# JuliaParallel/DistributedArrays.jl

Measured on AMD Instinct MI355X. Metric: sum(DArray) GB/s, higher is better.
Workload: dtype f64; 1 GPU; cfg2: sum(drand(Float64, 2^28)) per GPU, 1-D block distribution; per_gpu_elems=268435456, global_elems=268435456

## Files before the change

distributedarrays_jl_amd/csrc/abi.hip:

```cpp
#include "common.hpp"
#include <stdarg.h>
#include <stdio.h>
#include <stdlib.h>
#include <unistd.h>
#include <errno.h>
#include <time.h>

namespace da {

static State g_state;
State& st() { return g_state; }

char g_errbuf[1024] = "ok";

int set_err(int code, const char* fmt, ...) {
    va_list ap;
    va_start(ap, fmt);
    vsnprintf(g_errbuf, sizeof(g_errbuf), fmt, ap);
    va_end(ap);
    return code;
}

int ensure_scratch(size_t bytes) {
    if (st().scratch_bytes >= bytes) return 0;
    if (st().scratch) hipFree(st().scratch);
    st().scratch = nullptr;
    st().scratch_bytes = 0;
    DA_CHECK_HIP(hipMalloc(&st().scratch, bytes));
    st().scratch_bytes = bytes;
    return 0;
}

int ensure_partials(size_t bytes) {
    if (st().partials_bytes >= bytes) return 0;
    if (st().partials) hipFree(st().partials);
    st().partials = nullptr;
    st().partials_bytes = 0;
    DA_CHECK_HIP(hipMalloc(&st().partials, bytes));
    st().partials_bytes = bytes;
    return 0;
}

static ncclDataType_t nccl_dtype(int dtype) {
    switch (dtype) {
    case DA_F64: return ncclDouble;
    case DA_F32: return ncclFloat;
    default: return ncclInt64;
    }
}

static ncclRedOp_t nccl_redop(int redop) {
    switch (redop) {
    case DA_RED_ADD: return ncclSum;
    case DA_RED_MUL: return ncclProd;
    case DA_RED_MIN: return ncclMin;
    default: return ncclMax;
    }
}

}

using namespace da;

extern "C" {

static uint64_t round_sz(uint64_t nbytes);
static int pool_trim_locked();


int da_init(int device, int rank, int nranks, const char* rccl_uid_path) {
    if (st().inited) return 0;
    if (nranks < 1 || rank < 0 || rank >= nranks)
        return set_err(-2, "da_init: bad rank %d/%d", rank, nranks);
    DA_CHECK_HIP(hipSetDevice(device));
    DA_CHECK_HIP(hipStreamCreateWithFlags(&st().stream, hipStreamNonBlocking));
    DA_CHECK_HIP(hipStreamCreateWithFlags(&st().comm_stream,
                                          hipStreamNonBlocking));
    DA_CHECK_HIP(hipEventCreateWithFlags(&st().ev_main,
                                         hipEventDisableTiming));
    DA_CHECK_HIP(hipEventCreateWithFlags(&st().ev_comm,
                                         hipEventDisableTiming));
    DA_CHECK_HIP(hipMalloc(&st().red_ticket, sizeof(unsigned int)));
    DA_CHECK_HIP(hipMemset(st().red_ticket, 0, sizeof(unsigned int)));
    st().device = device;
    st().rank = rank;
    st().nranks = nranks;
    if (nranks > 1) {
        if (!rccl_uid_path)
            return set_err(-2, "da_init: nranks>1 needs a uid path");
        ncclUniqueId uid;
        if (rank == 0) {
            DA_CHECK_NCCL(ncclGetUniqueId(&uid));
            char tmp[1024];
            snprintf(tmp, sizeof(tmp), "%s.tmp", rccl_uid_path);
            FILE* f = fopen(tmp, "wb");
            if (!f) return set_err(-4, "da_init: cannot write %s", tmp);
            fwrite(&uid, sizeof(uid), 1, f);
            fclose(f);
            if (rename(tmp, rccl_uid_path) != 0)
                return set_err(-4, "da_init: rename failed: %s",
                               strerror(errno));
        } else {
            FILE* f = nullptr;
            for (int i = 0; i < 1200 && !f; ++i) {
                f = fopen(rccl_uid_path, "rb");
                if (!f) usleep(100000);
            }
            if (!f) return set_err(-4, "da_init: uid file never appeared");
            size_t got = fread(&uid, 1, sizeof(uid), f);
            fclose(f);
            if (got != sizeof(uid))
                return set_err(-4, "da_init: short uid file");
        }
        DA_CHECK_NCCL(ncclCommInitRank(&st().comm, nranks, uid, rank));
    }
    st().inited = true;
    return 0;
}

int da_shutdown(void) {
    if (!st().inited) return 0;
    if (st().comm) { ncclCommDestroy(st().comm); st().comm = nullptr; }
    if (st().scratch) { hipFree(st().scratch); st().scratch = nullptr; }
    if (st().partials) { hipFree(st().partials); st().partials = nullptr; }
    (void)copy_nd_release();
    st().scratch_bytes = st().partials_bytes = 0;
    {
        std::lock_guard<std::mutex> g(st().mem_mtx);
        for (auto& kv : st().allocs) (void)hipFree(kv.first);
        st().allocs.clear();
        st().bytes_in_use = 0;
        (void)pool_trim_locked();
    }
    if (st().red_ticket) { (void)hipFree(st().red_ticket);
                           st().red_ticket = nullptr; }
    if (st().ev_main) { (void)hipEventDestroy(st().ev_main); st().ev_main = nullptr; }
    if (st().ev_comm) { (void)hipEventDestroy(st().ev_comm); st().ev_comm = nullptr; }
    if (st().comm_stream) { (void)hipStreamDestroy(st().comm_stream);
                            st().comm_stream = nullptr; }
    if (st().stream) { (void)hipStreamDestroy(st().stream); st().stream = nullptr; }
    st().inited = false;
    return 0;
}

int da_rank(void) { return st().rank; }
int da_nranks(void) { return st().nranks; }


static uint64_t round_sz(uint64_t nbytes) {
    if (nbytes == 0) nbytes = 1;
    return (nbytes + 255) & ~(uint64_t)255;
}

static int pool_trim_locked() {
    for (auto& kv : st().pool)
        for (void* p : kv.second)
            if (hipFree(p) != hipSuccess)
                return set_err(-5, "da_pool_trim: hipFree failed");
    st().pool.clear();
    st().pool_bytes = 0;
    return 0;
}

int da_alloc(uint64_t nbytes, int dtype, void** chunk) {
    DA_REQUIRE_INIT();
    if (!chunk) return set_err(-3, "da_alloc: null out");
    (void)dtype;
    uint64_t sz = round_sz(nbytes);
    void* p = nullptr;
    {
        std::lock_guard<std::mutex> g(st().mem_mtx);
        auto it = st().pool.find(sz);
        if (it != st().pool.end() && !it->second.empty()) {
            p = it->second.back();
            it->second.pop_back();
            st().pool_bytes -= sz;
        }
    }
    if (!p) {
        hipError_t e = hipMalloc(&p, sz);
        if (e != hipSuccess) {
            std::lock_guard<std::mutex> g(st().mem_mtx);
            int rc = pool_trim_locked();
            if (rc) return rc;
            e = hipMalloc(&p, sz);
            if (e != hipSuccess)
                return set_err(-(1000 + (int)e), "da_alloc(%llu): %s",
                               (unsigned long long)sz,
                               hipGetErrorString(e));
        }
    }
    {
        std::lock_guard<std::mutex> g(st().mem_mtx);
        st().allocs[p] = sz;
        st().bytes_in_use += sz;
    }
    *chunk = p;
    return 0;
}

int da_free(void* chunk) {
    DA_REQUIRE_INIT();
    if (!chunk) return 0;
    std::lock_guard<std::mutex> g(st().mem_mtx);
    auto it = st().allocs.find(chunk);
    if (it == st().allocs.end())
        return set_err(-3, "da_free: unknown chunk %p", chunk);
    uint64_t sz = it->second;
    st().bytes_in_use -= sz;
    st().allocs.erase(it);
    st().pool[sz].push_back(chunk);
    st().pool_bytes += sz;
    return 0;
}

int da_pool_trim(void) {
    DA_REQUIRE_INIT();
    DA_CHECK_HIP(hipStreamSynchronize(st().stream));
    std::lock_guard<std::mutex> g(st().mem_mtx);
    return pool_trim_locked();
}

uint64_t da_pool_bytes(void) {
    std::lock_guard<std::mutex> g(st().mem_mtx);
    return st().pool_bytes;
}

uint64_t da_bytes_in_use(void) {
    std::lock_guard<std::mutex> g(st().mem_mtx);
    return st().bytes_in_use;
}

int da_h2d(void* chunk, const void* host, uint64_t nbytes) {
    DA_REQUIRE_INIT();
    DA_CHECK_HIP(hipMemcpyAsync(chunk, host, nbytes, hipMemcpyHostToDevice,
                                st().stream));
    DA_CHECK_HIP(hipStreamSynchronize(st().stream));
    return 0;
}

int da_d2h(const void* chunk, void* host, uint64_t nbytes) {
    DA_REQUIRE_INIT();
    DA_CHECK_HIP(hipMemcpyAsync(host, chunk, nbytes, hipMemcpyDeviceToHost,
                                st().stream));
    DA_CHECK_HIP(hipStreamSynchronize(st().stream));
    return 0;
}

int da_d2d(void* dst, const void* src, uint64_t nbytes) {
    DA_REQUIRE_INIT();
    DA_CHECK_HIP(hipMemcpyAsync(dst, src, nbytes, hipMemcpyDeviceToDevice,
                                st().stream));
    return 0;
}

int da_copy2d(void* dst, uint64_t dpitch, const void* src, uint64_t spitch,
              uint64_t width, uint64_t height) {
    DA_REQUIRE_INIT();
    DA_CHECK_HIP(hipMemcpy2DAsync(dst, dpitch, src, spitch, width, height,
                                  hipMemcpyDeviceToDevice, st().stream));
    return 0;
}

int da_copy_nd_plan(const uint64_t* dst_shape, const int64_t* dst_start,
                    const int64_t* dst_step, const int64_t* const* dst_idx,
                    const uint64_t* src_shape, const int64_t* src_start,
                    const int64_t* src_step, const int64_t* const* src_idx,
                    const uint64_t* count, int nd, int dtype) {
    return copy_nd_plan(dst_shape, dst_start, dst_step, dst_idx,
                        src_shape, src_start, src_step, src_idx,
                        count, nd, dtype);
}

int da_copy_nd(void* dst, const uint64_t* dst_shape, const int64_t* dst_start,
               const int64_t* dst_step, const int64_t* const* dst_idx,
               const void* src, const uint64_t* src_shape,
               const int64_t* src_start, const int64_t* src_step,
               const int64_t* const* src_idx,
               const uint64_t* count, int nd, int dtype) {
    DA_REQUIRE_INIT();
    return launch_copy_nd(dst, dst_shape, dst_start, dst_step, dst_idx,
                          src, src_shape, src_start, src_step, src_idx,
                          count, nd, dtype, st().stream);
}


int da_fill(void* chunk, double v, uint64_t n, int dtype) {
    DA_REQUIRE_INIT();
    return launch_fill(chunk, v, n, dtype, st().stream);
}

int da_rand(void* chunk, uint64_t n, int dtype, uint64_t seed, int kind,
            uint64_t offset) {
    DA_REQUIRE_INIT();
    return launch_rand(chunk, n, dtype, seed, kind, offset, st().stream);
}

int da_map(int opcode, void* dst, const void* src, uint64_t n, int dtype) {
    DA_REQUIRE_INIT();
    return launch_map(opcode, dst, src, n, dtype, st().stream);
}

int da_map2(int opcode, void* dst, const void* a, const void* b,
            uint64_t n, int dtype) {
    DA_REQUIRE_INIT();
    return launch_map2(opcode, dst, a, b, n, dtype, st().stream);
}

int da_map2_scalar(int opcode, void* dst, const void* src, double c,
                   int reverse, uint64_t n, int dtype) {
    DA_REQUIRE_INIT();
    return launch_map2_scalar(opcode, dst, src, c, reverse, n, dtype,
                              st().stream);
}

int da_bcast_fma(void* d, const void* a, const void* b, double c,
                 uint64_t n, int dtype) {
    DA_REQUIRE_INIT();
    return launch_bcast_fma(d, a, b, c, n, dtype, st().stream);
}

int da_expr(const int32_t* prog, int prog_len, void* dst,
            const uint64_t* dst_dims, int nd,
            void* const* srcs, const uint64_t* src_strides, int nsrcs,
            const double* consts, int nconsts, uint64_t n, int dtype) {
    DA_REQUIRE_INIT();
    return launch_expr(prog, prog_len, dst, dst_dims, nd, srcs,
                       src_strides, nsrcs, consts, nconsts, n, dtype,
                       st().stream);
}

int da_expr_jit_state(void) { return expr_jit_state(); }
const char* da_expr_jit_errstr(void) { return expr_jit_err(); }

int da_axpby(void* y, const void* x, double alpha, double beta,
             uint64_t n, int dtype) {
    DA_REQUIRE_INIT();
    return launch_axpby(y, x, alpha, beta, n, dtype, st().stream);
}

int da_add(void* dest, const void* src, double scale, uint64_t n, int dtype) {
    DA_REQUIRE_INIT();
    return launch_add(dest, src, scale, n, dtype, st().stream);
}

int da_scale(void* a, double s, uint64_t n, int dtype) {
    DA_REQUIRE_INIT();
    return launch_scale(a, s, n, dtype, st().stream);
}

int da_cast(void* dst, int dst_dtype, const void* src, int src_dtype,
            uint64_t n) {
    DA_REQUIRE_INIT();
    return launch_cast(dst, dst_dtype, src, src_dtype, n, st().stream);
}

int da_reduce(int mapop, int redop, const void* src, uint64_t n, int dtype,
              void* out) {
    DA_REQUIRE_INIT();
    return launch_reduce(mapop, redop, src, n, dtype, out, st().stream);
}

int da_count(int mapop, const void* src, uint64_t n, int dtype,
             int64_t* out) {
    DA_REQUIRE_INIT();
    return launch_count(mapop, src, n, dtype, out, st().stream);
}

int da_reduce_dims(int mapop, int redop, const void* src, uint64_t inner,
                   uint64_t axis, uint64_t outer, int dtype, void* dst) {
    DA_REQUIRE_INIT();
    return launch_reduce_dims(mapop, redop, src, inner, axis, outer,
                              dtype, dst, st().stream);
}

int da_allreduce(void* inout, int count, int dtype, int redop) {
    DA_REQUIRE_INIT();
    if (count <= 0) return set_err(-3, "da_allreduce: bad count");
    size_t bytes = (size_t)count * dtype_size(dtype);
    if (st().nranks == 1) return 0;
    int rc = ensure_scratch(bytes);
    if (rc) return rc;
    DA_CHECK_HIP(hipMemcpyAsync(st().scratch, inout, bytes,
                                hipMemcpyHostToDevice, st().stream));
    DA_CHECK_NCCL(ncclAllReduce(st().scratch, st().scratch, count,
                                nccl_dtype(dtype), nccl_redop(redop),
                                st().comm, st().stream));
    DA_CHECK_HIP(hipMemcpyAsync(inout, st().scratch, bytes,
                                hipMemcpyDeviceToHost, st().stream));
    DA_CHECK_HIP(hipStreamSynchronize(st().stream));
    return 0;
}


int da_gemm_f64(void* C, const void* A, const void* B,
                int64_t m, int64_t n, int64_t k,
                int64_t lda, int64_t ldb, int64_t ldc,
                double alpha, double beta) {
    DA_REQUIRE_INIT();
    return launch_gemm_f64(C, A, B, m, n, k, lda, ldb, ldc, alpha, beta,
                           st().stream);
}

int da_gemm_f32(void* C, const void* A, const void* B,
                int64_t m, int64_t n, int64_t k,
                int64_t lda, int64_t ldb, int64_t ldc,
                double alpha, double beta) {
    DA_REQUIRE_INIT();
    return launch_gemm_f32(C, A, B, m, n, k, lda, ldb, ldc, alpha, beta,
                           st().stream);
}

int da_gemm_i64(void* C, const void* A, const void* B,
                int64_t m, int64_t n, int64_t k,
                int64_t lda, int64_t ldb, int64_t ldc,
                int64_t alpha, int64_t beta) {
    DA_REQUIRE_INIT();
    return launch_gemm_i64(C, A, B, m, n, k, lda, ldb, ldc, alpha, beta,
                           st().stream);
}

int da_transpose(void* dst, const void* src, uint64_t m, uint64_t n,
                 int dtype) {
    DA_REQUIRE_INIT();
    return launch_transpose(dst, src, m, n, dtype, st().stream);
}

int da_diag_scale(void* a, uint64_t m, uint64_t n, const void* diag,
                  int side, int dtype) {
    DA_REQUIRE_INIT();
    return launch_diag_scale(a, m, n, diag, side, dtype, st().stream);
}

int dbg_mfma_probe_f64(const void* A, const void* B, void* out_c,
                       void* out_raw) {
    DA_REQUIRE_INIT();
    return dbg_mfma_probe_impl(DA_F64, A, B, out_c, out_raw, st().stream);
}
// ... 160 lines not shown
```

distributedarrays_jl_amd/csrc/common.hpp:

```cpp
#pragma once
#include <hip/hip_runtime.h>
#include <rccl/rccl.h>
#include <stdint.h>
#include <stdio.h>
#include <string.h>
#include <mutex>
#include <unordered_map>

#include "darray_hip.h"

namespace da {

struct State {
    bool inited = false;
    int device = 0;
    int rank = 0;
    int nranks = 1;
    hipStream_t stream = nullptr;
    hipStream_t comm_stream = nullptr;
    bool p2p_comm = false;
    hipEvent_t ev_main = nullptr, ev_comm = nullptr;
    ncclComm_t comm = nullptr;
    void* scratch = nullptr;
    size_t scratch_bytes = 0;
    void* partials = nullptr;
    size_t partials_bytes = 0;
    unsigned int* red_ticket = nullptr;
    std::mutex mem_mtx;
    std::unordered_map<void*, uint64_t> allocs;
    uint64_t bytes_in_use = 0;
    std::unordered_map<uint64_t, std::vector<void*>> pool;
    uint64_t pool_bytes = 0;
};

State& st();

extern char g_errbuf[1024];
int set_err(int code, const char* fmt, ...);

#define DA_CHECK_HIP(expr) do {                                          \
    hipError_t _e = (expr);                                              \
    if (_e != hipSuccess)                                                \
        return da::set_err(-(1000 + (int)_e), "%s:%d hip error: %s",     \
                           __FILE__, __LINE__, hipGetErrorString(_e));   \
} while (0)

#define DA_CHECK_NCCL(expr) do {                                         \
    ncclResult_t _e = (expr);                                            \
    if (_e != ncclSuccess)                                               \
        return da::set_err(-(2000 + (int)_e), "%s:%d rccl error: %s",    \
                           __FILE__, __LINE__, ncclGetErrorString(_e));  \
} while (0)

#define DA_REQUIRE_INIT() do {                                           \
    if (!da::st().inited)                                                \
        return da::set_err(-1, "libdarray_hip: da_init() not called");   \
} while (0)

inline size_t dtype_size(int dtype) {
    switch (dtype) {
        case DA_F64: return 8;
        case DA_F32: return 4;
        case DA_I64: return 8;
    }
    return 0;
}

int ensure_scratch(size_t bytes);
int ensure_partials(size_t bytes);

int launch_fill(void* chunk, double v, uint64_t n, int dtype, hipStream_t s);
int launch_rand(void* chunk, uint64_t n, int dtype, uint64_t seed, int kind,
                uint64_t offset, hipStream_t s);
int launch_map(int opcode, void* dst, const void* src, uint64_t n, int dtype,
               hipStream_t s);
int launch_map2(int opcode, void* dst, const void* a, const void* b,
                uint64_t n, int dtype, hipStream_t s);
int launch_bcast_fma(void* d, const void* a, const void* b, double c,
                     uint64_t n, int dtype, hipStream_t s);
int launch_map2_scalar(int opcode, void* dst, const void* src, double c,
                       int rev, uint64_t n, int dtype, hipStream_t s);
int launch_expr(const int32_t* prog, int plen, void* dst,
                const uint64_t* dst_dims, int nd,
                void* const* srcs, const uint64_t* src_strides, int nsrcs,
                const double* consts, int nconsts,
                uint64_t n, int dtype, hipStream_t s);
int launch_expr_jit(const int32_t* prog, int plen, void* dst,
                    const uint64_t* dst_dims, int nd,
                    void* const* srcs, const uint64_t* src_strides,
                    int nsrcs, const double* consts, int nconsts,
                    uint64_t n, int dtype, hipStream_t s);
int expr_jit_state();
const char* expr_jit_err();
int launch_transpose(void* dst, const void* src, uint64_t m, uint64_t n,
                     int dtype, hipStream_t s);
int launch_diag_scale(void* a, uint64_t m, uint64_t n, const void* diag,
                      int side, int dtype, hipStream_t s);
int launch_axpby(void* y, const void* x, double alpha, double beta,
                 uint64_t n, int dtype, hipStream_t s);
int launch_add(void* dest, const void* src, double scale, uint64_t n,
               int dtype, hipStream_t s);
int launch_scale(void* a, double s_, uint64_t n, int dtype, hipStream_t s);
int launch_cast(void* dst, int dst_dtype, const void* src, int src_dtype,
                uint64_t n, hipStream_t s);
int launch_reduce(int mapop, int redop, const void* src, uint64_t n,
                  int dtype, void* out_host, hipStream_t s);
int launch_count(int mapop, const void* src, uint64_t n, int dtype,
                 int64_t* out_host, hipStream_t s);
int launch_reduce_dims(int mapop, int redop, const void* src,
                       uint64_t inner, uint64_t axis, uint64_t outer,
                       int dtype, void* dst, hipStream_t s);
int launch_gemm_f64(void* C, const void* A, const void* B,
                    int64_t m, int64_t n, int64_t k,
                    int64_t lda, int64_t ldb, int64_t ldc,
                    double alpha, double beta, hipStream_t s);
int launch_gemm_i64(void* C, const void* A, const void* B,
                    int64_t m, int64_t n, int64_t k,
                    int64_t lda, int64_t ldb, int64_t ldc,
                    int64_t alpha, int64_t beta, hipStream_t s);
int launch_gemm_f32(void* C, const void* A, const void* B,
                    int64_t m, int64_t n, int64_t k,
                    int64_t lda, int64_t ldb, int64_t ldc,
                    double alpha, double beta, hipStream_t s);
int copy_nd_plan(const uint64_t* dst_shape, const int64_t* dst_start,
                 const int64_t* dst_step, const int64_t* const* dst_idx,
                 const uint64_t* src_shape, const int64_t* src_start,
                 const int64_t* src_step, const int64_t* const* src_idx,
                 const uint64_t* count, int nd, int dtype);
int launch_copy_nd(void* dst, const uint64_t* dst_shape,
                   const int64_t* dst_start, const int64_t* dst_step,
                   const int64_t* const* dst_idx,
                   const void* src, const uint64_t* src_shape,
                   const int64_t* src_start, const int64_t* src_step,
                   const int64_t* const* src_idx,
                   const uint64_t* count, int nd, int dtype, hipStream_t s);
int copy_nd_release();
int reduce_dims_variant(uint64_t inner, uint64_t axis, uint64_t outer);
int gemm_path(int64_t m, int64_t n, int64_t k);
int dbg_mfma_probe_impl(int dtype, const void* A, const void* B,
                        void* out_c, void* out_raw, hipStream_t s);

}
```

distributedarrays_jl_amd/csrc/kernels_reduce.hip:

```cpp
#include "common.hpp"
#include <stdlib.h>

namespace da {

constexpr int RTPB = 256;
constexpr int RMAXB = 8192;

static inline int reduce_grid(uint64_t want) {
    static int cap = -1;
    if (cap < 0) {
        const char* e = getenv("DA_RBLOCKS");
        cap = e ? atoi(e) : 2048;
        if (cap < 1 || cap > RMAXB) cap = 2048;
    }
    if (want < 1) want = 1;
    return (int)(want > (uint64_t)cap ? (uint64_t)cap : want);
}

static inline bool reduce_v4() {
    static int v = -1;
    if (v < 0) {
        const char* e = getenv("DA_RV4");
        v = e ? atoi(e) : 0;
    }
    return v == 1;
}

template <typename T> struct RedIdent {
    static __device__ __host__ T get(int redop) {
        switch (redop) {
        case DA_RED_ADD: return (T)0;
        case DA_RED_MUL: return (T)1;
        case DA_RED_MIN: return (T)INFINITY;
        case DA_RED_MAX: return (T)(-INFINITY);
        }
        return (T)0;
    }
};
template <> struct RedIdent<int64_t> {
    static __device__ __host__ int64_t get(int redop) {
        switch (redop) {
        case DA_RED_ADD: return 0;
        case DA_RED_MUL: return 1;
        case DA_RED_MIN: return INT64_MAX;
        case DA_RED_MAX: return INT64_MIN;
        }
        return 0;
    }
};

template <typename T>
__device__ __forceinline__ T red_comb(int redop, T a, T b) {
    switch (redop) {
    case DA_RED_ADD: return a + b;
    case DA_RED_MUL: return a * b;
    case DA_RED_MIN:
        return a != a ? a : (b != b ? b : (a < b ? a : b));
    case DA_RED_MAX:
        return a != a ? a : (b != b ? b : (a > b ? a : b));
    }
    return a;
}
__device__ __forceinline__ int64_t red_comb(int redop, int64_t a, int64_t b) {
    switch (redop) {
    case DA_RED_ADD: return (int64_t)((uint64_t)a + (uint64_t)b);
    case DA_RED_MUL: return (int64_t)((uint64_t)a * (uint64_t)b);
    case DA_RED_MIN: return a < b ? a : b;
    case DA_RED_MAX: return a > b ? a : b;
    }
    return a;
}

template <typename T>
__device__ __forceinline__ T mapf(int mapop, T x) {
    switch (mapop) {
    case DA_REDF_IDENTITY: return x;
    case DA_REDF_ABS: return fabs(x);
    case DA_REDF_ABS2: return x * x;
    case DA_REDF_ISNAN: return (T)(x != x ? 1 : 0);
    case DA_REDF_ISFINITE: return (T)(isfinite((double)x) ? 1 : 0);
    case DA_REDF_NONZERO: return (T)(x != (T)0 ? 1 : 0);
    }
    return x;
}
__device__ __forceinline__ int64_t mapf(int mapop, int64_t x) {
    switch (mapop) {
    case DA_REDF_IDENTITY: return x;
    case DA_REDF_ABS: return x < 0 ? (int64_t)(0ull - (uint64_t)x) : x;
    case DA_REDF_ABS2: return (int64_t)((uint64_t)x * (uint64_t)x);
    case DA_REDF_ISNAN: return 0;
    case DA_REDF_ISFINITE: return 1;
    case DA_REDF_NONZERO: return x != 0 ? 1 : 0;
    }
    return x;
}

template <typename T>
__device__ __forceinline__ T block_reduce(int redop, T v) {
    __shared__ T lds[RTPB / 64];
#pragma unroll
    for (int off = 32; off > 0; off >>= 1)
        v = red_comb(redop, v, (T)__shfl_down(v, off, 64));
    int wave = threadIdx.x / 64, lane = threadIdx.x % 64;
    if (lane == 0) lds[wave] = v;
    __syncthreads();
    if (wave == 0) {
        T w = lane < (RTPB / 64) ? lds[lane]
                                 : RedIdent<T>::get(redop);
#pragma unroll
        for (int off = 2; off > 0; off >>= 1)
            w = red_comb(redop, w, (T)__shfl_down(w, off, 64));
        return w;
    }
    return v;
}

template <typename T, int MOP = -1, int ROP = -1>
__global__ void reduce_stage1(int mapop, int redop, const T* __restrict__ src,
                              uint64_t n, T* __restrict__ partials) {
    if (MOP >= 0) mapop = MOP;
    if (ROP >= 0) redop = ROP;
    uint64_t i = (uint64_t)blockIdx.x * blockDim.x + threadIdx.x;
    uint64_t stride = (uint64_t)gridDim.x * blockDim.x;
    T acc = RedIdent<T>::get(redop);
    using V = T __attribute__((ext_vector_type(2)));
    uint64_t nv = n / 2;
    const V* sv = reinterpret_cast<const V*>(src);
    for (uint64_t j = i; j < nv; j += stride) {
        V v = sv[j];
        acc = red_comb(redop, acc, mapf<T>(mapop, (T)v.x));
        acc = red_comb(redop, acc, mapf<T>(mapop, (T)v.y));
    }
    for (uint64_t j = 2 * nv + i; j < n; j += stride)
        acc = red_comb(redop, acc, mapf<T>(mapop, src[j]));
    acc = block_reduce(redop, acc);
    if (threadIdx.x == 0) partials[blockIdx.x] = acc;
}

template <typename T, int MOP = -1, int ROP = -1>
__global__ void reduce_stage1_v4(int mapop, int redop,
                                 const T* __restrict__ src, uint64_t n,
                                 T* __restrict__ partials) {
    if (MOP >= 0) mapop = MOP;
    if (ROP >= 0) redop = ROP;
    uint64_t i = (uint64_t)blockIdx.x * blockDim.x + threadIdx.x;
    uint64_t stride = (uint64_t)gridDim.x * blockDim.x;
    T acc = RedIdent<T>::get(redop);
    using V = T __attribute__((ext_vector_type(4)));
    uint64_t nv = n / 4;
    const V* sv = reinterpret_cast<const V*>(src);
    for (uint64_t j = i; j < nv; j += stride) {
        V v = sv[j];
        acc = red_comb(redop, acc, mapf<T>(mapop, (T)v.x));
        acc = red_comb(redop, acc, mapf<T>(mapop, (T)v.y));
        acc = red_comb(redop, acc, mapf<T>(mapop, (T)v.z));
        acc = red_comb(redop, acc, mapf<T>(mapop, (T)v.w));
    }
    for (uint64_t j = 4 * nv + i; j < n; j += stride)
        acc = red_comb(redop, acc, mapf<T>(mapop, src[j]));
    acc = block_reduce(redop, acc);
    if (threadIdx.x == 0) partials[blockIdx.x] = acc;
}

template <typename T>
__global__ void reduce_fused(int mapop, int redop, const T* __restrict__ src,
                             uint64_t n, T* __restrict__ partials,
                             unsigned int* __restrict__ ticket,
                             T* __restrict__ out) {
    __shared__ int is_last;
    uint64_t i = (uint64_t)blockIdx.x * blockDim.x + threadIdx.x;
    uint64_t stride = (uint64_t)gridDim.x * blockDim.x;
    T acc = RedIdent<T>::get(redop);
    using V = T __attribute__((ext_vector_type(2)));
    uint64_t nv = n / 2;
    const V* sv = reinterpret_cast<const V*>(src);
    for (uint64_t j = i; j < nv; j += stride) {
        V v = sv[j];
        acc = red_comb(redop, acc, mapf<T>(mapop, (T)v.x));
        acc = red_comb(redop, acc, mapf<T>(mapop, (T)v.y));
    }
    for (uint64_t j = 2 * nv + i; j < n; j += stride)
        acc = red_comb(redop, acc, mapf<T>(mapop, src[j]));
    acc = block_reduce(redop, acc);
    if (threadIdx.x == 0) partials[blockIdx.x] = acc;
    __asm__ volatile("s_waitcnt vmcnt(0)" ::: "memory");
    __syncthreads();
    if (threadIdx.x == 0) {
        __builtin_amdgcn_fence(__ATOMIC_RELEASE, "agent");
        __asm__ volatile("s_waitcnt vmcnt(0)" ::: "memory");
        unsigned int t = __hip_atomic_fetch_add(
            ticket, 1u, __ATOMIC_RELAXED, __HIP_MEMORY_SCOPE_AGENT);
        is_last = (t == gridDim.x - 1);
    }
    __syncthreads();
    if (!is_last) return;
    if (threadIdx.x == 0)
        __builtin_amdgcn_fence(__ATOMIC_ACQUIRE, "agent");
    __syncthreads();
    T facc = RedIdent<T>::get(redop);
    for (unsigned int j = threadIdx.x; j < gridDim.x; j += blockDim.x)
        facc = red_comb(redop, facc, partials[j]);
    __syncthreads();
    facc = block_reduce(redop, facc);
    if (threadIdx.x == 0) {
        out[0] = facc;
        *ticket = 0;
    }
}

template <typename T>
__global__ void reduce_stage2(int redop, const T* __restrict__ partials,
                              int np, T* __restrict__ out) {
    T acc = RedIdent<T>::get(redop);
    for (int j = threadIdx.x; j < np; j += blockDim.x)
        acc = red_comb(redop, acc, partials[j]);
    acc = block_reduce(redop, acc);
    if (threadIdx.x == 0) out[0] = acc;
}

template <typename T>
static int do_reduce(int mapop, int redop, const T* src, uint64_t n,
                     void* out_host, hipStream_t s) {
    if (n == 0) {
        *(T*)out_host = RedIdent<T>::get(redop);
        return 0;
    }
    bool v4 = reduce_v4();
    uint64_t want = (n / (v4 ? 4 : 2) + RTPB - 1) / RTPB;
    int g = reduce_grid(want);
    int rc = ensure_partials((RMAXB + 1) * sizeof(double));
    if (rc) return rc;
    T* parts = (T*)st().partials;
    T* dout = (T*)((double*)st().partials + RMAXB);
    unsigned int* ticket = st().red_ticket;
    static int fused = -1;
    if (fused < 0) {
        const char* e = getenv("DA_RED_FUSED");
        fused = e ? atoi(e) : 0;
    }
    if (fused && !v4) {
        hipLaunchKernelGGL(reduce_fused<T>, dim3(g), dim3(RTPB), 0, s,
                           mapop, redop, src, n, parts, ticket, dout);
        DA_CHECK_HIP(hipGetLastError());
    } else {
        if (v4)
            hipLaunchKernelGGL((reduce_stage1_v4<T>), dim3(g), dim3(RTPB),
                               0, s, mapop, redop, src, n, parts);
        else if (mapop == DA_REDF_IDENTITY && redop == DA_RED_ADD)
            hipLaunchKernelGGL((reduce_stage1<T, DA_REDF_IDENTITY,
                                DA_RED_ADD>), dim3(g), dim3(RTPB), 0, s,
                               mapop, redop, src, n, parts);
        else if (mapop == DA_REDF_ABS2 && redop == DA_RED_ADD)
            hipLaunchKernelGGL((reduce_stage1<T, DA_REDF_ABS2,
                                DA_RED_ADD>), dim3(g), dim3(RTPB), 0, s,
                               mapop, redop, src, n, parts);
        else if (mapop == DA_REDF_ABS && redop == DA_RED_ADD)
            hipLaunchKernelGGL((reduce_stage1<T, DA_REDF_ABS,
                                DA_RED_ADD>), dim3(g), dim3(RTPB), 0, s,
                               mapop, redop, src, n, parts);
        else if (mapop == DA_REDF_IDENTITY && redop == DA_RED_MAX)
            hipLaunchKernelGGL((reduce_stage1<T, DA_REDF_IDENTITY,
                                DA_RED_MAX>), dim3(g), dim3(RTPB), 0, s,
                               mapop, redop, src, n, parts);
        else if (mapop == DA_REDF_IDENTITY && redop == DA_RED_MIN)
            hipLaunchKernelGGL((reduce_stage1<T, DA_REDF_IDENTITY,
                                DA_RED_MIN>), dim3(g), dim3(RTPB), 0, s,
                               mapop, redop, src, n, parts);
        else
            hipLaunchKernelGGL((reduce_stage1<T>), dim3(g), dim3(RTPB),
                               0, s, mapop, redop, src, n, parts);
        DA_CHECK_HIP(hipGetLastError());
        hipLaunchKernelGGL(reduce_stage2<T>, dim3(1), dim3(RTPB), 0, s,
                           redop, parts, g, dout);
        DA_CHECK_HIP(hipGetLastError());
    }
    DA_CHECK_HIP(hipMemcpyAsync(out_host, dout, sizeof(T),
                                hipMemcpyDeviceToHost, s));
    DA_CHECK_HIP(hipStreamSynchronize(s));
    return 0;
}

template <typename T>
__device__ __forceinline__ int64_t predf(int mapop, T x) {
    switch (mapop) {
    case DA_REDF_ISNAN: return x != x ? 1 : 0;
    case DA_REDF_ISFINITE: return isfinite((double)x) ? 1 : 0;
    }
    return x != (T)0 ? 1 : 0;
}
template <>
__device__ __forceinline__ int64_t predf<int64_t>(int mapop, int64_t x) {
    return mapf(mapop, x);
}

template <typename T>
__global__ void count_stage1(int mapop, const T* __restrict__ src,
                             uint64_t n, int64_t* __restrict__ partials) {
    uint64_t i = (uint64_t)blockIdx.x * blockDim.x + threadIdx.x;
    uint64_t stride = (uint64_t)gridDim.x * blockDim.x;
    int64_t acc = 0;
    using V = T __attribute__((ext_vector_type(2)));
    uint64_t nv = n / 2;
    const V* sv = reinterpret_cast<const V*>(src);
    for (uint64_t j = i; j < nv; j += stride) {
        V v = sv[j];
        acc += predf<T>(mapop, (T)v.x) + predf<T>(mapop, (T)v.y);
    }
    for (uint64_t j = 2 * nv + i; j < n; j += stride)
        acc += predf<T>(mapop, src[j]);
    acc = block_reduce(DA_RED_ADD, acc);
    if (threadIdx.x == 0) partials[blockIdx.x] = acc;
}

template <typename T>
static int do_count(int mapop, const T* src, uint64_t n, int64_t* out_host,
                    hipStream_t s) {
    int g = reduce_grid((n / 2 + RTPB - 1) / RTPB);
    int rc = ensure_partials((RMAXB + 1) * sizeof(double));
    if (rc) return rc;
    int64_t* parts = (int64_t*)st().partials;
    int64_t* dout = parts + RMAXB;
    hipLaunchKernelGGL(count_stage1<T>, dim3(g), dim3(RTPB), 0, s,
                       mapop, src, n, parts);
    DA_CHECK_HIP(hipGetLastError());
    hipLaunchKernelGGL(reduce_stage2<int64_t>, dim3(1), dim3(RTPB), 0, s,
                       (int)DA_RED_ADD, parts, g, dout);
    DA_CHECK_HIP(hipGetLastError());
    DA_CHECK_HIP(hipMemcpyAsync(out_host, dout, sizeof(int64_t),
                                hipMemcpyDeviceToHost, s));
    DA_CHECK_HIP(hipStreamSynchronize(s));
    return 0;
}

int launch_count(int mapop, const void* src, uint64_t n, int dtype,
                 int64_t* out_host, hipStream_t s) {
    if (mapop < DA_REDF_ISNAN || mapop > DA_REDF_NONZERO)
        return set_err(-3, "da_count: mapop %d is not a predicate", mapop);
    if (!out_host) return set_err(-3, "da_count: null out");
    if (dtype != DA_F64 && dtype != DA_F32 && dtype != DA_I64)
        return set_err(-3, "da_count: bad dtype %d", dtype);
    if (n == 0) { *out_host = 0; return 0; }
    switch (dtype) {
    case DA_F64: return do_count<double>(mapop, (const double*)src, n,
                                         out_host, s);
    case DA_F32: return do_count<float>(mapop, (const float*)src, n,
                                        out_host, s);
    }
    return do_count<int64_t>(mapop, (const int64_t*)src, n, out_host, s);
}

template <typename T, int MOP, int ROP>
__global__ void reduce_dims_threads(int mapop, int redop,
                                    const T* __restrict__ src,
                                    uint64_t inner, uint64_t axis,
                                    uint64_t outer, T* __restrict__ dst) {
    const int mop_ = MOP >= 0 ? MOP : mapop;
    const int rop_ = ROP >= 0 ? ROP : redop;
    uint64_t t = (uint64_t)blockIdx.x * blockDim.x + threadIdx.x;
    uint64_t stride = (uint64_t)gridDim.x * blockDim.x;
    uint64_t total = inner * outer;
    for (uint64_t e = t; e < total; e += stride) {
        uint64_t i = e % inner, o = e / inner;
        const T* p = src + i + o * inner * axis;
        T acc = RedIdent<T>::get(rop_);
        for (uint64_t a = 0; a < axis; ++a)
            acc = red_comb(rop_, acc, mapf(mop_, p[a * inner]));
        dst[i + o * inner] = acc;
    }
}

template <typename T, int MOP, int ROP>
__global__ void reduce_dims_waves(int mapop, int redop,
                                  const T* __restrict__ src,
                                  uint64_t inner, uint64_t axis,
                                  uint64_t outer, T* __restrict__ dst) {
    const int mop_ = MOP >= 0 ? MOP : mapop;
    const int rop_ = ROP >= 0 ? ROP : redop;
    uint64_t wid = ((uint64_t)blockIdx.x * blockDim.x + threadIdx.x) / 64;
    uint64_t nw = ((uint64_t)gridDim.x * blockDim.x) / 64;
    int lane = threadIdx.x & 63;
    uint64_t total = inner * outer;
    for (uint64_t e = wid; e < total; e += nw) {
        uint64_t i = e % inner, o = e / inner;
        const T* p = src + i + o * inner * axis;
        T acc = RedIdent<T>::get(rop_);
        for (uint64_t a = lane; a < axis; a += 64)
            acc = red_comb(rop_, acc, mapf(mop_, p[a * inner]));
#pragma unroll
        for (int off = 32; off > 0; off >>= 1)
            acc = red_comb(rop_, acc, (T)__shfl_down(acc, off, 64));
        if (lane == 0) dst[i + o * inner] = acc;
    }
}

template <typename T, int MOP, int ROP>
__global__ void reduce_dims_blocks(int mapop, int redop,
                                   const T* __restrict__ src,
                                   uint64_t inner, uint64_t axis,
                                   uint64_t outer, T* __restrict__ dst) {
    const int mop_ = MOP >= 0 ? MOP : mapop;
    const int rop_ = ROP >= 0 ? ROP : redop;
    uint64_t total = inner * outer;
    for (uint64_t e = blockIdx.x; e < total; e += gridDim.x) {
        uint64_t i = e % inner, o = e / inner;
        const T* p = src + i + o * inner * axis;
        T acc = RedIdent<T>::get(rop_);
        for (uint64_t a = threadIdx.x; a < axis; a += blockDim.x)
            acc = red_comb(rop_, acc, mapf(mop_, p[a * inner]));
        acc = block_reduce(rop_, acc);
        if (threadIdx.x == 0) dst[i + o * inner] = acc;
        __syncthreads();
    }
}

template <typename T, int MOP, int ROP>
__global__ void reduce_dims_slices1(int mapop, int redop,
                                    const T* __restrict__ src,
                                    uint64_t inner, uint64_t axis,
                                    int nb, T* __restrict__ partials) {
    const int mop_ = MOP >= 0 ? MOP : mapop;
    const int rop_ = ROP >= 0 ? ROP : redop;
    uint64_t o = blockIdx.z;
    const T* base = src + o * inner * axis;
    uint64_t row = (uint64_t)blockIdx.x * blockDim.x + threadIdx.x;
    if (row >= inner) return;
    uint64_t a0 = axis * blockIdx.y / nb;
    uint64_t a1 = axis * (blockIdx.y + 1) / nb;
    T acc = RedIdent<T>::get(rop_);
    for (uint64_t a = a0; a < a1; ++a)
        acc = red_comb(rop_, acc, mapf(mop_, base[row + a * inner]));
    partials[(o * nb + blockIdx.y) * inner + row] = acc;
}

template <typename T>
__global__ void reduce_dims_slices2(int redop, const T* __restrict__ partials,
                                    uint64_t inner, int nb,
                                    T* __restrict__ dst, uint64_t outer) {
    uint64_t e = (uint64_t)blockIdx.x * blockDim.x + threadIdx.x;
    uint64_t stride = (uint64_t)gridDim.x * blockDim.x;
    for (uint64_t t = e; t < inner * outer; t += stride) {
        uint64_t row = t % inner, o = t / inner;
        T acc = RedIdent<T>::get(redop);
        for (int b = 0; b < nb; ++b)
            acc = red_comb(redop, acc,
                           partials[(o * nb + b) * inner + row]);
        dst[row + o * inner] = acc;
    }
}

int reduce_dims_variant(uint64_t inner, uint64_t axis, uint64_t outer) {
    uint64_t total = inner * outer;
    if (total < 262144 && inner >= 64 && axis >= 64 && outer <= 64)
        return DA_DIMS_SLICES;
    if (total >= 262144 && inner >= 64)
        return DA_DIMS_THREADS;
    if (inner < 64 && axis >= 64 && total >= 16384)
        return DA_DIMS_WAVES;
    return DA_DIMS_BLOCKS;
}

template <typename T, int MOP, int ROP>
static int do_reduce_dims_t(int mapop, int redop, const T* src,
                            uint64_t inner, uint64_t axis, uint64_t outer,
                            T* dst, hipStream_t s) {
    uint64_t total = inner * outer;
    if (total == 0) return 0;
    const int variant = reduce_dims_variant(inner, axis, outer);
    if (variant == DA_DIMS_SLICES) {
        uint64_t row_tiles = (inner + RTPB - 1) / RTPB;
        int nb = (int)(2048 / row_tiles);
        if (nb < 1) nb = 1;
        if (nb > 64) nb = 64;
        if ((uint64_t)nb > axis) nb = (int)axis;
        int rc = ensure_partials((uint64_t)nb * inner * outer * sizeof(T));
        if (rc) return rc;
        T* parts = (T*)st().partials;
        dim3 g((inner + RTPB - 1) / RTPB, nb, outer);
        hipLaunchKernelGGL((reduce_dims_slices1<T, MOP, ROP>), g,
                           dim3(RTPB), 0, s,
                           mapop, redop, src, inner, axis, nb, parts);
        DA_CHECK_HIP(hipGetLastError());
        uint64_t want = (total + RTPB - 1) / RTPB;
        int g2 = (int)(want < 1 ? 1 : (want > 2048 ? 2048 : want));
        hipLaunchKernelGGL(reduce_dims_slices2<T>, dim3(g2), dim3(RTPB), 0,
                           s, redop, parts, inner, nb, dst, outer);
        DA_CHECK_HIP(hipGetLastError());
        return 0;
    }
    if (variant == DA_DIMS_THREADS) {
        uint64_t want = (total + RTPB - 1) / RTPB;
        int g = (int)(want < 1 ? 1 : (want > 8192 ? 8192 : want));
        hipLaunchKernelGGL((reduce_dims_threads<T, MOP, ROP>), dim3(g),
                           dim3(RTPB), 0,
                           s, mapop, redop, src, inner, axis, outer, dst);
    } else if (variant == DA_DIMS_WAVES) {
        uint64_t want = (total * 64 + RTPB - 1) / RTPB;
        int g = (int)(want < 1 ? 1 : (want > 8192 ? 8192 : want));
        hipLaunchKernelGGL((reduce_dims_waves<T, MOP, ROP>), dim3(g),
                           dim3(RTPB), 0,
                           s, mapop, redop, src, inner, axis, outer, dst);
    } else {
        int g = (int)(total < 1 ? 1 : (total > 8192 ? 8192 : total));
        hipLaunchKernelGGL((reduce_dims_blocks<T, MOP, ROP>), dim3(g),
                           dim3(RTPB), 0,
                           s, mapop, redop, src, inner, axis, outer, dst);
    }
    DA_CHECK_HIP(hipGetLastError());
    return 0;
}

template <typename T>
static int do_reduce_dims(int mapop, int redop, const T* src,
                          uint64_t inner, uint64_t axis, uint64_t outer,
                          T* dst, hipStream_t s) {
    if (redop == DA_RED_ADD) {
        if (mapop == DA_REDF_IDENTITY)
            return do_reduce_dims_t<T, DA_REDF_IDENTITY, DA_RED_ADD>(
                mapop, redop, src, inner, axis, outer, dst, s);
        if (mapop == DA_REDF_ABS2)
            return do_reduce_dims_t<T, DA_REDF_ABS2, DA_RED_ADD>(
                mapop, redop, src, inner, axis, outer, dst, s);
    }
    if (redop == DA_RED_MAX && mapop == DA_REDF_IDENTITY)
        return do_reduce_dims_t<T, DA_REDF_IDENTITY, DA_RED_MAX>(
            mapop, redop, src, inner, axis, outer, dst, s);
    if (redop == DA_RED_MIN && mapop == DA_REDF_IDENTITY)
        return do_reduce_dims_t<T, DA_REDF_IDENTITY, DA_RED_MIN>(
            mapop, redop, src, inner, axis, outer, dst, s);
    return do_reduce_dims_t<T, -1, -1>(mapop, redop, src, inner, axis,
                                       outer, dst, s);
}

int launch_reduce_dims(int mapop, int redop, const void* src,
                       uint64_t inner, uint64_t axis, uint64_t outer,
                       int dtype, void* dst, hipStream_t s) {
    if (mapop < 0 || mapop > DA_REDF_NONZERO || redop < 0 || redop > DA_RED_MAX)
        return set_err(-3, "da_reduce_dims: bad op (%d,%d)", mapop, redop);
    switch (dtype) {
    case DA_F64: return do_reduce_dims<double>(mapop, redop,
        (const double*)src, inner, axis, outer, (double*)dst, s);
    case DA_F32: return do_reduce_dims<float>(mapop, redop,
        (const float*)src, inner, axis, outer, (float*)dst, s);
    case DA_I64: return do_reduce_dims<int64_t>(mapop, redop,
        (const int64_t*)src, inner, axis, outer, (int64_t*)dst, s);
    }
    return set_err(-3, "da_reduce_dims: bad dtype %d", dtype);
}

int launch_reduce(int mapop, int redop, const void* src, uint64_t n,
                  int dtype, void* out_host, hipStream_t s) {
    if (mapop < 0 || mapop > DA_REDF_NONZERO || redop < 0 || redop > DA_RED_MAX)
        return set_err(-3, "da_reduce: bad op (%d,%d)", mapop, redop);
    switch (dtype) {
    case DA_F64: return do_reduce<double>(mapop, redop, (const double*)src,
                                          n, out_host, s);
    case DA_F32: return do_reduce<float>(mapop, redop, (const float*)src,
                                         n, out_host, s);
    case DA_I64: return do_reduce<int64_t>(mapop, redop, (const int64_t*)src,
                                           n, out_host, s);
    }
    return set_err(-3, "da_reduce: bad dtype %d", dtype);
}

}
```

Measured before the change: 6023 GB/s.

## Default to fused single-pass reduction with monotonic ticket and pinned host result

```diff
diff --git a/distributedarrays_jl_amd/csrc/abi.hip b/distributedarrays_jl_amd/csrc/abi.hip
--- a/distributedarrays_jl_amd/csrc/abi.hip
+++ b/distributedarrays_jl_amd/csrc/abi.hip
@@ -82,6 +82,11 @@
                                          hipEventDisableTiming));
     DA_CHECK_HIP(hipMalloc(&st().red_ticket, sizeof(unsigned int)));
     DA_CHECK_HIP(hipMemset(st().red_ticket, 0, sizeof(unsigned int)));
+    st().red_base = 0;
+    DA_CHECK_HIP(hipHostMalloc(&st().red_host, 16, hipHostMallocDefault));
+    memset(st().red_host, 0, 16);
+    DA_CHECK_HIP(hipHostGetDevicePointer(&st().red_host_dev,
+                                         st().red_host, 0));
     st().device = device;
     st().rank = rank;
     st().nranks = nranks;
@@ -134,6 +139,8 @@
     }
     if (st().red_ticket) { (void)hipFree(st().red_ticket);
                            st().red_ticket = nullptr; }
+    if (st().red_host) { (void)hipHostFree(st().red_host);
+                         st().red_host = st().red_host_dev = nullptr; }
     if (st().ev_main) { (void)hipEventDestroy(st().ev_main); st().ev_main = nullptr; }
     if (st().ev_comm) { (void)hipEventDestroy(st().ev_comm); st().ev_comm = nullptr; }
     if (st().comm_stream) { (void)hipStreamDestroy(st().comm_stream);
diff --git a/distributedarrays_jl_amd/csrc/common.hpp b/distributedarrays_jl_amd/csrc/common.hpp
--- a/distributedarrays_jl_amd/csrc/common.hpp
+++ b/distributedarrays_jl_amd/csrc/common.hpp
@@ -26,6 +26,9 @@
     void* partials = nullptr;
     size_t partials_bytes = 0;
     unsigned int* red_ticket = nullptr;
+    unsigned int red_base = 0;
+    void* red_host = nullptr;
+    void* red_host_dev = nullptr;
     std::mutex mem_mtx;
     std::unordered_map<void*, uint64_t> allocs;
     uint64_t bytes_in_use = 0;
diff --git a/distributedarrays_jl_amd/csrc/kernels_reduce.hip b/distributedarrays_jl_amd/csrc/kernels_reduce.hip
--- a/distributedarrays_jl_amd/csrc/kernels_reduce.hip
+++ b/distributedarrays_jl_amd/csrc/kernels_reduce.hip
@@ -96,8 +96,7 @@
 }
 
 template <typename T>
-__device__ __forceinline__ T block_reduce(int redop, T v) {
-    __shared__ T lds[RTPB / 64];
+__device__ __forceinline__ T block_reduce_in(int redop, T v, T* lds) {
 #pragma unroll
     for (int off = 32; off > 0; off >>= 1)
         v = red_comb(redop, v, (T)__shfl_down(v, off, 64));
@@ -115,24 +114,37 @@
     return v;
 }
 
+template <typename T>
+__device__ __forceinline__ T block_reduce(int redop, T v) {
+    __shared__ T lds[RTPB / 64];
+    return block_reduce_in(redop, v, lds);
+}
+
+template <int W, typename T, typename A, typename F>
+__device__ __forceinline__ A grid_accumulate(const T* __restrict__ src,
+                                             uint64_t n, A acc, F fold) {
+    uint64_t i = (uint64_t)blockIdx.x * RTPB + threadIdx.x;
+    uint64_t stride = (uint64_t)gridDim.x * RTPB;
+    using V = T __attribute__((ext_vector_type(W)));
+    uint64_t nv = n / W;
+    const V* sv = reinterpret_cast<const V*>(src);
+    for (uint64_t j = i; j < nv; j += stride) {
+        V v = sv[j];
+#pragma unroll
+        for (int k = 0; k < W; ++k) acc = fold(acc, (T)v[k]);
+    }
+    for (uint64_t j = W * nv + i; j < n; j += stride)
+        acc = fold(acc, src[j]);
+    return acc;
+}
+
 template <typename T, int MOP = -1, int ROP = -1>
 __global__ void reduce_stage1(int mapop, int redop, const T* __restrict__ src,
                               uint64_t n, T* __restrict__ partials) {
     if (MOP >= 0) mapop = MOP;
     if (ROP >= 0) redop = ROP;
-    uint64_t i = (uint64_t)blockIdx.x * blockDim.x + threadIdx.x;
-    uint64_t stride = (uint64_t)gridDim.x * blockDim.x;
-    T acc = RedIdent<T>::get(redop);
-    using V = T __attribute__((ext_vector_type(2)));
-    uint64_t nv = n / 2;
-    const V* sv = reinterpret_cast<const V*>(src);
-    for (uint64_t j = i; j < nv; j += stride) {
-        V v = sv[j];
-        acc = red_comb(redop, acc, mapf<T>(mapop, (T)v.x));
-        acc = red_comb(redop, acc, mapf<T>(mapop, (T)v.y));
-    }
-    for (uint64_t j = 2 * nv + i; j < n; j += stride)
-        acc = red_comb(redop, acc, mapf<T>(mapop, src[j]));
+    T acc = grid_accumulate<2>(src, n, RedIdent<T>::get(redop),
+        [=](T a, T x) { return red_comb(redop, a, mapf<T>(mapop, x)); });
     acc = block_reduce(redop, acc);
     if (threadIdx.x == 0) partials[blockIdx.x] = acc;
 }
@@ -143,69 +155,61 @@
                                  T* __restrict__ partials) {
     if (MOP >= 0) mapop = MOP;
     if (ROP >= 0) redop = ROP;
-    uint64_t i = (uint64_t)blockIdx.x * blockDim.x + threadIdx.x;
-    uint64_t stride = (uint64_t)gridDim.x * blockDim.x;
-    T acc = RedIdent<T>::get(redop);
-    using V = T __attribute__((ext_vector_type(4)));
-    uint64_t nv = n / 4;
-    const V* sv = reinterpret_cast<const V*>(src);
-    for (uint64_t j = i; j < nv; j += stride) {
-        V v = sv[j];
-        acc = red_comb(redop, acc, mapf<T>(mapop, (T)v.x));
-        acc = red_comb(redop, acc, mapf<T>(mapop, (T)v.y));
-        acc = red_comb(redop, acc, mapf<T>(mapop, (T)v.z));
-        acc = red_comb(redop, acc, mapf<T>(mapop, (T)v.w));
-    }
-    for (uint64_t j = 4 * nv + i; j < n; j += stride)
-        acc = red_comb(redop, acc, mapf<T>(mapop, src[j]));
+    T acc = grid_accumulate<4>(src, n, RedIdent<T>::get(redop),
+        [=](T a, T x) { return red_comb(redop, a, mapf<T>(mapop, x)); });
     acc = block_reduce(redop, acc);
     if (threadIdx.x == 0) partials[blockIdx.x] = acc;
 }
 
-template <typename T>
-__global__ void reduce_fused(int mapop, int redop, const T* __restrict__ src,
-                             uint64_t n, T* __restrict__ partials,
-                             unsigned int* __restrict__ ticket,
-                             T* __restrict__ out) {
-    __shared__ int is_last;
-    uint64_t i = (uint64_t)blockIdx.x * blockDim.x + threadIdx.x;
-    uint64_t stride = (uint64_t)gridDim.x * blockDim.x;
-    T acc = RedIdent<T>::get(redop);
-    using V = T __attribute__((ext_vector_type(2)));
-    uint64_t nv = n / 2;
-    const V* sv = reinterpret_cast<const V*>(src);
-    for (uint64_t j = i; j < nv; j += stride) {
-        V v = sv[j];
-        acc = red_comb(redop, acc, mapf<T>(mapop, (T)v.x));
-        acc = red_comb(redop, acc, mapf<T>(mapop, (T)v.y));
-    }
-    for (uint64_t j = 2 * nv + i; j < n; j += stride)
-        acc = red_comb(redop, acc, mapf<T>(mapop, src[j]));
-    acc = block_reduce(redop, acc);
-    if (threadIdx.x == 0) partials[blockIdx.x] = acc;
-    __asm__ volatile("s_waitcnt vmcnt(0)" ::: "memory");
-    __syncthreads();
+template <typename A>
+__device__ __forceinline__ void publish_partial(A* p, A v) {
+    if constexpr (sizeof(A) == 8)
+        __hip_atomic_store((unsigned long long*)p,
+                           __builtin_bit_cast(unsigned long long, v),
+                           __ATOMIC_RELAXED, __HIP_MEMORY_SCOPE_AGENT);
+    else
+        __hip_atomic_store((unsigned int*)p,
+                           __builtin_bit_cast(unsigned int, v),
+                           __ATOMIC_RELAXED, __HIP_MEMORY_SCOPE_AGENT);
+}
+
+template <typename A>
+__device__ __forceinline__ void fanin_finish(int redop, A acc, A* partials,
+                                             unsigned int* ticket,
+                                             unsigned int base, A* out,
+                                             A* sh) {
     if (threadIdx.x == 0) {
-        __builtin_amdgcn_fence(__ATOMIC_RELEASE, "agent");
+        publish_partial(partials + blockIdx.x, acc);
         __asm__ volatile("s_waitcnt vmcnt(0)" ::: "memory");
         unsigned int t = __hip_atomic_fetch_add(
             ticket, 1u, __ATOMIC_RELAXED, __HIP_MEMORY_SCOPE_AGENT);
-        is_last = (t == gridDim.x - 1);
+        sh[RTPB / 64] = (t - base == gridDim.x - 1) ? (A)1 : (A)0;
     }
     __syncthreads();
-    if (!is_last) return;
-    if (threadIdx.x == 0)
+    if (sh[RTPB / 64] == (A)0) return;
+    if (threadIdx.x == 0) {
         __builtin_amdgcn_fence(__ATOMIC_ACQUIRE, "agent");
+        __asm__ volatile("s_waitcnt vmcnt(0)" ::: "memory");
+    }
     __syncthreads();
-    T facc = RedIdent<T>::get(redop);
-    for (unsigned int j = threadIdx.x; j < gridDim.x; j += blockDim.x)
+    A facc = RedIdent<A>::get(redop);
+    for (unsigned int j = threadIdx.x; j < gridDim.x; j += RTPB)
         facc = red_comb(redop, facc, partials[j]);
-    __syncthreads();
-    facc = block_reduce(redop, facc);
-    if (threadIdx.x == 0) {
-        out[0] = facc;
-        *ticket = 0;
-    }
+    facc = block_reduce_in(redop, facc, sh);
+    if (threadIdx.x == 0) out[0] = facc;
+}
+
+template <typename T, int MOP = -1, int ROP = -1>
+__global__ void reduce_fused(int mapop, int redop, const T* __restrict__ src,
+                             uint64_t n, T* partials, unsigned int* ticket,
+                             unsigned int base, T* out) {
+    if (MOP >= 0) mapop = MOP;
+    if (ROP >= 0) redop = ROP;
+    __shared__ T sh[RTPB / 64 + 1];
+    T acc = grid_accumulate<2>(src, n, RedIdent<T>::get(redop),
+        [=](T a, T x) { return red_comb(redop, a, mapf<T>(mapop, x)); });
+    acc = block_reduce_in(redop, acc, sh);
+    fanin_finish(redop, acc, partials, ticket, base, out, sh);
 }
 
 template <typename T>
@@ -218,6 +222,36 @@
     if (threadIdx.x == 0) out[0] = acc;
 }
 
+static inline bool reduce_fused_on() {
+    static int v = -1;
+    if (v < 0) {
+        const char* e = getenv("DA_RED_FUSED");
+        v = e ? (atoi(e) != 0) : 1;
+    }
+    return v == 1;
+}
+
+template <typename T> struct FlatArgs {
+    bool fused;
+    int grid, mapop, redop;
+    const T* src;
+    uint64_t n;
+    T *parts, *out;
+    hipStream_t s;
+};
+
+template <typename T, int MOP, int ROP>
+static void launch_flat(const FlatArgs<T>& a) {
+    if (a.fused)
+        hipLaunchKernelGGL((reduce_fused<T, MOP, ROP>), dim3(a.grid),
+                           dim3(RTPB), 0, a.s, a.mapop, a.redop, a.src, a.n,
+                           a.parts, st().red_ticket, st().red_base, a.out);
+    else
+        hipLaunchKernelGGL((reduce_stage1<T, MOP, ROP>), dim3(a.grid),
+                           dim3(RTPB), 0, a.s, a.mapop, a.redop, a.src, a.n,
+                           a.parts);
+}
+
 template <typename T>
 static int do_reduce(int mapop, int redop, const T* src, uint64_t n,
                      void* out_host, hipStream_t s) {
@@ -228,55 +262,35 @@
     bool v4 = reduce_v4();
     uint64_t want = (n / (v4 ? 4 : 2) + RTPB - 1) / RTPB;
     int g = reduce_grid(want);
-    int rc = ensure_partials((RMAXB + 1) * sizeof(double));
+    int rc = ensure_partials(RMAXB * sizeof(double));
     if (rc) return rc;
-    T* parts = (T*)st().partials;
-    T* dout = (T*)((double*)st().partials + RMAXB);
-    unsigned int* ticket = st().red_ticket;
-    static int fused = -1;
-    if (fused < 0) {
-        const char* e = getenv("DA_RED_FUSED");
-        fused = e ? atoi(e) : 0;
-    }
-    if (fused && !v4) {
-        hipLaunchKernelGGL(reduce_fused<T>, dim3(g), dim3(RTPB), 0, s,
-                           mapop, redop, src, n, parts, ticket, dout);
+    FlatArgs<T> a = {reduce_fused_on() && !v4, g, mapop, redop, src, n,
+                     (T*)st().partials, (T*)st().red_host_dev, s};
+    if (v4)
+        hipLaunchKernelGGL((reduce_stage1_v4<T>), dim3(g), dim3(RTPB),
+                           0, s, mapop, redop, src, n, a.parts);
+    else if (mapop == DA_REDF_IDENTITY && redop == DA_RED_ADD)
+        launch_flat<T, DA_REDF_IDENTITY, DA_RED_ADD>(a);
+    else if (mapop == DA_REDF_ABS2 && redop == DA_RED_ADD)
+        launch_flat<T, DA_REDF_ABS2, DA_RED_ADD>(a);
+    else if (mapop == DA_REDF_ABS && redop == DA_RED_ADD)
+        launch_flat<T, DA_REDF_ABS, DA_RED_ADD>(a);
+    else if (mapop == DA_REDF_IDENTITY && redop == DA_RED_MAX)
+        launch_flat<T, DA_REDF_IDENTITY, DA_RED_MAX>(a);
+    else if (mapop == DA_REDF_IDENTITY && redop == DA_RED_MIN)
+        launch_flat<T, DA_REDF_IDENTITY, DA_RED_MIN>(a);
+    else
+        launch_flat<T, -1, -1>(a);
+    DA_CHECK_HIP(hipGetLastError());
+    if (a.fused) {
+        st().red_base += (unsigned int)g;
+    } else {
+        hipLaunchKernelGGL(reduce_stage2<T>, dim3(1), dim3(RTPB), 0, s,
+                           redop, a.parts, g, a.out);
         DA_CHECK_HIP(hipGetLastError());
-    } else {
-        if (v4)
-            hipLaunchKernelGGL((reduce_stage1_v4<T>), dim3(g), dim3(RTPB),
-                               0, s, mapop, redop, src, n, parts);
-        else if (mapop == DA_REDF_IDENTITY && redop == DA_RED_ADD)
-            hipLaunchKernelGGL((reduce_stage1<T, DA_REDF_IDENTITY,
-                                DA_RED_ADD>), dim3(g), dim3(RTPB), 0, s,
-                               mapop, redop, src, n, parts);
-        else if (mapop == DA_REDF_ABS2 && redop == DA_RED_ADD)
-            hipLaunchKernelGGL((reduce_stage1<T, DA_REDF_ABS2,
-                                DA_RED_ADD>), dim3(g), dim3(RTPB), 0, s,
-                               mapop, redop, src, n, parts);
-        else if (mapop == DA_REDF_ABS && redop == DA_RED_ADD)
-            hipLaunchKernelGGL((reduce_stage1<T, DA_REDF_ABS,
-                                DA_RED_ADD>), dim3(g), dim3(RTPB), 0, s,
-                               mapop, redop, src, n, parts);
-        else if (mapop == DA_REDF_IDENTITY && redop == DA_RED_MAX)
-            hipLaunchKernelGGL((reduce_stage1<T, DA_REDF_IDENTITY,
-                                DA_RED_MAX>), dim3(g), dim3(RTPB), 0, s,
-                               mapop, redop, src, n, parts);
-        else if (mapop == DA_REDF_IDENTITY && redop == DA_RED_MIN)
-            hipLaunchKernelGGL((reduce_stage1<T, DA_REDF_IDENTITY,
-                                DA_RED_MIN>), dim3(g), dim3(RTPB), 0, s,
-                               mapop, redop, src, n, parts);
-        else
-            hipLaunchKernelGGL((reduce_stage1<T>), dim3(g), dim3(RTPB),
-                               0, s, mapop, redop, src, n, parts);
-        DA_CHECK_HIP(hipGetLastError());
-        hipLaunchKernelGGL(reduce_stage2<T>, dim3(1), dim3(RTPB), 0, s,
-                           redop, parts, g, dout);
-        DA_CHECK_HIP(hipGetLastError());
-    }
-    DA_CHECK_HIP(hipMemcpyAsync(out_host, dout, sizeof(T),
-                                hipMemcpyDeviceToHost, s));
+    }
     DA_CHECK_HIP(hipStreamSynchronize(s));
+    memcpy(out_host, st().red_host, sizeof(T));
     return 0;
 }
 
@@ -296,39 +310,47 @@
 template <typename T>
 __global__ void count_stage1(int mapop, const T* __restrict__ src,
                              uint64_t n, int64_t* __restrict__ partials) {
-    uint64_t i = (uint64_t)blockIdx.x * blockDim.x + threadIdx.x;
-    uint64_t stride = (uint64_t)gridDim.x * blockDim.x;
-    int64_t acc = 0;
-    using V = T __attribute__((ext_vector_type(2)));
-    uint64_t nv = n / 2;
-    const V* sv = reinterpret_cast<const V*>(src);
-    for (uint64_t j = i; j < nv; j += stride) {
-        V v = sv[j];
-        acc += predf<T>(mapop, (T)v.x) + predf<T>(mapop, (T)v.y);
-    }
-    for (uint64_t j = 2 * nv + i; j < n; j += stride)
-        acc += predf<T>(mapop, src[j]);
+    int64_t acc = grid_accumulate<2>(src, n, (int64_t)0,
+        [=](int64_t a, T x) { return a + predf<T>(mapop, x); });
     acc = block_reduce(DA_RED_ADD, acc);
     if (threadIdx.x == 0) partials[blockIdx.x] = acc;
+}
+
+template <typename T>
+__global__ void count_fused(int mapop, const T* __restrict__ src, uint64_t n,
+                            int64_t* partials, unsigned int* ticket,
+                            unsigned int base, int64_t* out) {
+    __shared__ int64_t sh[RTPB / 64 + 1];
+    int64_t acc = grid_accumulate<2>(src, n, (int64_t)0,
+        [=](int64_t a, T x) { return a + predf<T>(mapop, x); });
+    acc = block_reduce_in((int)DA_RED_ADD, acc, sh);
+    fanin_finish((int)DA_RED_ADD, acc, partials, ticket, base, out, sh);
 }
 
 template <typename T>
 static int do_count(int mapop, const T* src, uint64_t n, int64_t* out_host,
                     hipStream_t s) {
     int g = reduce_grid((n / 2 + RTPB - 1) / RTPB);
-    int rc = ensure_partials((RMAXB + 1) * sizeof(double));
+    int rc = ensure_partials(RMAXB * sizeof(double));
     if (rc) return rc;
     int64_t* parts = (int64_t*)st().partials;
-    int64_t* dout = parts + RMAXB;
-    hipLaunchKernelGGL(count_stage1<T>, dim3(g), dim3(RTPB), 0, s,
-                       mapop, src, n, parts);
-    DA_CHECK_HIP(hipGetLastError());
-    hipLaunchKernelGGL(reduce_stage2<int64_t>, dim3(1), dim3(RTPB), 0, s,
-                       (int)DA_RED_ADD, parts, g, dout);
-    DA_CHECK_HIP(hipGetLastError());
-    DA_CHECK_HIP(hipMemcpyAsync(out_host, dout, sizeof(int64_t),
-                                hipMemcpyDeviceToHost, s));
+    int64_t* out = (int64_t*)st().red_host_dev;
+    if (reduce_fused_on()) {
+        hipLaunchKernelGGL(count_fused<T>, dim3(g), dim3(RTPB), 0, s,
+                           mapop, src, n, parts, st().red_ticket,
+                           st().red_base, out);
+        DA_CHECK_HIP(hipGetLastError());
+        st().red_base += (unsigned int)g;
+    } else {
+        hipLaunchKernelGGL(count_stage1<T>, dim3(g), dim3(RTPB), 0, s,
+                           mapop, src, n, parts);
+        DA_CHECK_HIP(hipGetLastError());
+        hipLaunchKernelGGL(reduce_stage2<int64_t>, dim3(1), dim3(RTPB), 0, s,
+                           (int)DA_RED_ADD, parts, g, out);
+        DA_CHECK_HIP(hipGetLastError());
+    }
     DA_CHECK_HIP(hipStreamSynchronize(s));
+    memcpy(out_host, st().red_host, sizeof(int64_t));
     return 0;
 }
 
```

Result: faster. 6178 GB/s (median of 6 runs) (+2.6%).
